# Cyan4973/FiniteStateEntropy

Hardware: NVIDIA H100
Metric: encode+decode GB/s (uncompressed) per GPU on 32 KB blocks; bit-exact vs ref (higher is better)
Workload: dtype u8

## Files before the change

finitestateentropy_b200/csrc/fse_dev.cuh:

```cuda
#pragma once
#include "common.cuh"

namespace fseb {

__device__ __forceinline__ unsigned hibit0(unsigned v) { return v ? hibit(v) : 0u; }

__device__ inline unsigned d_min_tablelog(u64 srcSize, unsigned msv)
{
    unsigned const bySrc = hibit0((u32)srcSize) + 1, bySym = hibit0(msv) + 2;
    return bySrc < bySym ? bySrc : bySym;
}

__device__ inline unsigned d_optimal_tablelog(unsigned maxTableLog, u64 srcSize, unsigned msv, unsigned minus)
{
    unsigned const bySrc = hibit0((u32)(srcSize - 1)) - minus;
    unsigned const floorBits = d_min_tablelog(srcSize, msv);
    unsigned tl = maxTableLog ? maxTableLog : FSE_DEF_TLOG;
    if (bySrc < tl) tl = bySrc;
    if (floorBits > tl) tl = floorBits;
    if (tl < FSE_MIN_TLOG) tl = FSE_MIN_TLOG;
    if (tl > FSE_MAX_TLOG) tl = FSE_MAX_TLOG;
    return tl;
}

// ... 149 lines not shown
            if (upto > *msvPtr) return err(E_MSV_TOO_SMALL);
            while (sym < upto) norm[sym++] = 0;
            if ((ip <= end - 7) || (ip + (held >> 3) <= end - 4)) { ip += held >> 3; held &= 7; bits = rd32(in + ip) >> held; }
            else bits >>= 2;
        }
        int const cut = (2 * threshold - 1) - remaining;
        int v;
        if ((bits & (u32)(threshold - 1)) < (u32)cut) { v = (int)(bits & (u32)(threshold - 1)); held += width - 1; }
        else { v = (int)(bits & (u32)(2 * threshold - 1)); if (v >= threshold) v -= cut; held += width; }
        v--;
        remaining -= v < 0 ? -v : v;
        norm[sym++] = (short)v;
        afterZero = !v;
        while (remaining < threshold) { width--; threshold >>= 1; }
        if ((ip <= end - 7) || (ip + (held >> 3) <= end - 4)) { ip += held >> 3; held &= 7; }
        else { held -= (int)(8 * (end - 4 - ip)); ip = end - 4; }
        bits = rd32(in + ip) >> (held & 31);
    }
    if (remaining != 1) return err(E_CORRUPT);
    if (held > 32) return err(E_CORRUPT);
    *msvPtr = sym - 1;
    ip += (held + 7) >> 3;
    if (padded && (u64)ip > trueSize) return err(E_CORRUPT);
    return (u64)ip;
}

__device__ inline bool d_spread_serial(u16* cellSym, const short* norm, unsigned msv, unsigned tl)
{
    u32 const size = 1u << tl, mask = size - 1;
    u32 const stride = (size >> 1) + (size >> 3) + 3;
    u32 high = size - 1, pos = 0;
    for (u32 s = 0; s <= msv; s++) if (norm[s] == -1) cellSym[high--] = (u16)s;
    for (u32 s = 0; s <= msv; s++) {
        int const n = norm[s];
        for (int k = 0; k < n; k++) {
            cellSym[pos] = (u16)s;
            do pos = (pos + stride) & mask; while (pos > high);
        }
    }
    return pos == 0;
}

__device__ inline void d_build_ctable_serial(u32* ct, const short* norm, unsigned msv, unsigned tl, u16* cellSym, u32* start)
{
    u32 const size = 1u << tl;
    u16* const hdr = (u16*)ct;
    u16* const next = hdr + 2;
    u32* const tt = ct + 1 + (tl ? (size >> 1) : 1);
    hdr[0] = (u16)tl; hdr[1] = (u16)msv;
    start[0] = 0;
    for (u32 s = 1; s <= msv + 1; s++) start[s] = start[s - 1] + (u32)(norm[s - 1] == -1 ? 1 : norm[s - 1]);
    start[msv + 1] = size + 1;
    d_spread_serial(cellSym, norm, msv, tl);
    for (u32 u = 0; u < size; u++) next[start[cellSym[u]]++] = (u16)(size + u);
    u32 total = 0;
    for (u32 s = 0; s <= msv; s++) {
        int const n = norm[s];
        if (n == 0) { tt[2 * s + 1] = ((tl + 1) << 16) - size; tt[2 * s] = 0; continue; }
        if (n == -1 || n == 1) { tt[2 * s + 1] = (tl << 16) - size; tt[2 * s] = total - 1; total++; }
        else {
            u32 const maxOut = tl - hibit((u32)n - 1);
            tt[2 * s + 1] = (maxOut << 16) - ((u32)n << maxOut);
            tt[2 * s] = total - (u32)n; total += (u32)n;
        }
    }
}

template <bool WIDE>
__device__ inline u64 d_build_dtable_serial(u32* dt, const short* norm, unsigned msv, unsigned tl,
                                            unsigned msvLimit, unsigned tlLimit, u16* cellSym, u16* nextOf)
{
    u32 const size = 1u << tl;
    unsigned fast = 1;
    if (msv > msvLimit) return err(E_MSV_TOO_LARGE);
    if (tl > tlLimit) return err(E_TLOG_TOO_LARGE);
    for (u32 s = 0; s <= msv; s++) {
        if (norm[s] == -1) nextOf[s] = 1;
        else { if (norm[s] >= (short)(1 << (tl - 1))) fast = 0; nextOf[s] = (u16)norm[s]; }
    }
    dt[0] = tl | (fast << 16);
    if (!d_spread_serial(cellSym, norm, msv, tl)) return err(E_GENERIC);
    for (u32 u = 0; u < size; u++) {
        u32 const sym = cellSym[u];
        u32 const x = nextOf[sym]++;
        u32 const nb = tl - hibit(x);
        u32 const ns = ((x << nb) - size) & 0xFFFF;
        dt[1 + u] = WIDE ? (ns | (nb << 16) | (sym << 20)) : (ns | (sym << 16) | (nb << 24));
    }
    return 0;
}

}
```

finitestateentropy_b200/csrc/huf_build_dev.cuh:

```cuda
#pragma once
#include "common.cuh"
#include "fse_dev.cuh"
#include "sink_dev.cuh"

namespace fseb {

struct HNode { u32 count; u16 parent; u8 sym; u8 len; };

struct HNodeView {
    HNode* p;
    __device__ u32 count(int i) const { return p[i].count; }
    __device__ u32 len(int i) const { return p[i].len; }
    __device__ void set_len(int i, u32 v) const { p[i].len = (u8)v; }
};
struct PackedNodeView {
    u32* p; int stride;
    __device__ u32 count(int i) const { return p[i * stride] & 0xFFFFFFu; }
    __device__ u32 len(int i) const { return p[i * stride] >> 24; }
    __device__ void set_len(int i, u32 v) const { u32& x = p[i * stride]; x = (x & 0xFFFFFFu) | (v << 24); }
};

template <class Nodes>
__device__ inline u32 d_huf_limit_depth(Nodes nd, u32 last, u32 maxBits)
{
    u32 const deepest = nd.len(last);
    if (deepest <= maxBits) return deepest;
    int debt = 0;
    u32 const unit = 1u << (deepest - maxBits);
    int n = (int)last;
    u32 const NONE = 0xF0F0F0F0u;
    u32 lastOfRank[HUF_MAX_TLOG + 2];
    while (nd.len(n) > maxBits) {
        debt += (int)(unit - (1u << (deepest - nd.len(n))));
        nd.set_len(n, maxBits); n--;
    }
    while (nd.len(n) == maxBits) n--;
    debt >>= (deepest - maxBits);
    for (u32 i = 0; i < HUF_MAX_TLOG + 2; i++) lastOfRank[i] = NONE;
    {   u32 cur = maxBits;
        for (int pos = n; pos >= 0; pos--) {
            if (nd.len(pos) >= cur) continue;
            cur = nd.len(pos);
            lastOfRank[maxBits - cur] = (u32)pos;
        }
    }
    while (debt > 0) {
        u32 dec = hibit((u32)debt) + 1;
        for (; dec > 1; dec--) {
            u32 const hi = lastOfRank[dec], lo = lastOfRank[dec - 1];
            if (hi == NONE) continue;
            if (lo == NONE) break;
            if (nd.count(hi) <= 2 * nd.count(lo)) break;
        }
        while (dec <= HUF_MAX_TLOG && lastOfRank[dec] == NONE) dec++;
        debt -= 1 << (dec - 1);
        if (lastOfRank[dec - 1] == NONE) lastOfRank[dec - 1] = lastOfRank[dec];
        nd.set_len(lastOfRank[dec], nd.len(lastOfRank[dec]) + 1);
        if (lastOfRank[dec] == 0) lastOfRank[dec] = NONE;
        else {
            lastOfRank[dec]--;
// ... 65 lines not shown
    u32 const mb = s_ret;
    if (mb > HUF_MAX_TLOG) return err(E_GENERIC);
    if ((u32)tid <= msv) lenOf[nd[tid].sym] = nd[tid].len;
    __syncthreads();
    if ((u32)tid <= msv) {
        u32 const len = lenOf[tid];
        u32 before = 0;
        for (u32 jj = 0; jj < (u32)tid; jj++) before += (lenOf[jj] == len);
        ctable[tid] = ((firstVal[len] + before) & 0xFFFF) | (len << 16);
    } else ctable[tid & 255] = 0;
    __syncthreads();
    return mb;
}

__device__ __forceinline__ void warp_sort256_desc(u32 (&key)[8], unsigned lane)
{
    #pragma unroll
    for (u32 k = 2; k <= 256; k <<= 1) {
        #pragma unroll
        for (u32 j = k >> 1; j > 0; j >>= 1) {
            if (j >= 32) {
                u32 const dj = j >> 5;
                #pragma unroll
                for (u32 i = 0; i < 8; i++) {
                    if (i & dj) continue;
                    u32 const e = i * 32;
                    bool const desc = (k == 256) || ((e & k) != 0) ;
                    u32 const lo = min(key[i], key[i | dj]), hi = max(key[i], key[i | dj]);
                    key[i] = desc ? hi : lo; key[i | dj] = desc ? lo : hi;
                }
            } else {
                #pragma unroll
                for (u32 i = 0; i < 8; i++) {
                    u32 const e = i * 32 + lane;
                    u32 const other = __shfl_xor_sync(0xFFFFFFFFu, key[i], j);
                    bool const asc = (k == 256) ? false : ((e & k) == 0);
                    bool const takeMin = ((e & j) == 0) == asc;
                    key[i] = takeMin ? min(key[i], other) : max(key[i], other);
                }
            }
        }
    }
}

__device__ inline u64 d_huf_compress_weights(u8* out, u64 cap, const u8* w, u64 n, u32* wksp)
{
    unsigned* const count = wksp;
    short* const norm = (short*)(wksp + 16);
    u32* const ct = wksp + 24;
    u16* const cellSym = (u16*)(wksp + 84);
    u32* const start = wksp + 116;
    unsigned msv = HUF_MAX_TLOG, tl = 6, best = 0;
    if (n <= 1) return 0;
    for (unsigned i = 0; i <= HUF_MAX_TLOG; i++) count[i] = 0;
    for (u64 i = 0; i < n; i++) count[w[i]]++;
    while (!count[msv]) msv--;
    for (unsigned s = 0; s <= msv; s++) best = count[s] > best ? count[s] : best;
    if (best == n) return 1;
    if (best == 1) return 0;
    tl = d_optimal_tablelog(tl, n, msv, 2);
    u64 r = d_normalize(norm, tl, count, n, msv); if (is_err(r)) return r;
    r = d_write_ncount(out, cap, norm, msv, tl); if (is_err(r)) return r;
    u64 const o = r;
    d_build_ctable_serial(ct, norm, msv, tl, cellSym, start);
    r = d_fse_encode_serial(out + o, cap - o, w, n, ct);
    if (r == 0) return 0;
    return o + r;
}

template <class CTable>
__device__ inline u64 d_huf_write_ctable(u8* out, u64 cap, CTable ctable, unsigned msv, unsigned huffLog, u32* wksp)
{
    u8* const weight = (u8*)(wksp + 160);
    if (msv > HUF_MAX_SV) return err(E_MSV_TOO_LARGE);
    for (unsigned n = 0; n < msv; n++) {
        unsigned const len = (ctable[n] >> 16) & 0xFF;
        weight[n] = (u8)(len ? huffLog + 1 - len : 0);
    }
    {   u64 const h = d_huf_compress_weights(out + 1, cap - 1, weight, msv, wksp);
        if (is_err(h)) return h;
        if ((h > 1) & (h < msv / 2)) { out[0] = (u8)h; return h + 1; }
    }
    if (msv > 128) return err(E_GENERIC);
    if (((msv + 1) / 2) + 1 > cap) return err(E_DST_TOO_SMALL);
    out[0] = (u8)(128 + (msv - 1));
    weight[msv] = 0;
    for (unsigned n = 0; n < msv; n += 2) out[(n / 2) + 1] = (u8)((weight[n] << 4) + weight[n + 1]);
    return ((msv + 1) / 2) + 1;
}

}
```

finitestateentropy_b200/csrc/huf_encode.cu:

```cuda
#include <mutex>
#include <type_traits>
#include <vector>
#include "common.cuh"
#include "launchers.h"
#include "launch_util.cuh"
#include "fse_dev.cuh"
#include "sink_dev.cuh"
#include "huf_build_dev.cuh"
#include "pack_dev.cuh"

namespace fseb {
namespace hufe {

constexpr unsigned FULL = 0xFFFFFFFFu;

struct __align__(16) Plan {
    u32 ctable[256];
    u8  header[136];
    u32 hSize;
    u32 state;
    u32 total;
    u32 streamOff[4];
    u32 streamBytes[4];
    u16 segCount[4][256];
};
enum : u32 { PLAN_EMIT = 0, PLAN_FINAL = 1, PLAN_EMIT_1X = 2 };

constexpr int PLAN_WARPS = 8;
constexpr u32 GROUP = 32;
constexpr u32 HDR_STRIDE = 34 + 224 + 1;
constexpr u32 CT_ROW = HDR_STRIDE;
constexpr u32 ROWS = CT_ROW + 256;
constexpr u32 NODE_END = 0x7FFFFFFFu, LEAF_END = 0xFFFFFFFFu;
struct PlanCta {
    u32 nd[ROWS][GROUP];
    u8  sym[256][GROUP];
    u64 res[GROUP];
    u16 msv[GROUP];
    u8  last[GROUP];
    u8  tlog[GROUP];
    u8  live[GROUP];
};
static_assert(ROWS >= 1 + 256 + PLAN_WARPS * 4 * 256 / GROUP, "segment histograms must fit in the rows above the leaves");
static_assert(ROWS >= 1 + 511 && CT_ROW >= 1 + 256, "node rows");
static_assert(HUF_BLOCK_MAX < (1u << 24), "node counts share a word with an 8-bit parent / length");
static_assert(sizeof(PlanCta) <= 76 * 1024, "three CTAs per SM");

template <int NS, class Count>
__device__ __forceinline__ void stream_bits(const u32 (&cell)[8], Count count, u32 (&bits)[NS])
{
    #pragma unroll
    for (int k = 0; k < NS; k++) {
        u32 acc = 0;
        #pragma unroll
        for (u32 i = 0; i < 8; i++) acc += count(k, i) * (cell[i] >> 16);
        #pragma unroll
        for (int dlt = 16; dlt; dlt >>= 1) acc += __shfl_xor_sync(FULL, acc, dlt);
        bits[k] = acc;
    }
}

template <int NS>
__device__ __forceinline__ bool place_streams(const u32 (&bits)[NS], u64 hs, u64 capLeft, u32 (&offs)[NS], u32 (&lens)[NS], u64& total)
{
    u64 op = (NS == 4) ? 6 : 0; bool fits = true;
    #pragma unroll
    for (int t = 0; t < NS; t++) {
        u64 const capk = capLeft - op;
        u64 const tot = (u64)bits[t] + 1;
        if (fits && (capk <= 8 || (tot >> 3) >= capk - 8)) fits = false;
        offs[t] = (u32)(hs + op); lens[t] = (u32)((tot + 7) >> 3);
        op += lens[t];
    }
    total = hs + op;
    return fits;
}

template <int NS, class Count>
__device__ __forceinline__ bool plan_streams(Plan& P, const u32 (&cell)[8], Count count, const u8* hdr, u64 hs, u64 cap, u32 n,
                                             unsigned lane, u64& total)
{
    u32 bits[NS], offs[NS], lens[NS];
    stream_bits<NS>(cell, count, bits);
// ... 54 lines not shown
    }
    for (u32 k = i + lane; k < end; k += 32) atomicAdd(&cnt[s[k]], 1u);
}

__device__ __forceinline__ void warp_hist4_pipelined(u32 (*count4)[256], const u8* s, u32 n, u32 seg, unsigned lane)
{
    const uint4* const gv = reinterpret_cast<const uint4*>(s) + lane;
    u32 const B = n / 2048, perSeg = seg / 2048;
    auto load = [&](uint4 (&x)[4], u32 b) {
        #pragma unroll
        for (int h = 0; h < 4; h++) x[h] = __ldg(gv + b * 128 + 32 * h);
    };
    auto count = [&](const uint4 (&x)[4], u32 b) {
        u32* const cnt = count4[b / perSeg];
        #pragma unroll
        for (int h = 0; h < 4; h++) {
            u32 const wd[4] = { x[h].x, x[h].y, x[h].z, x[h].w };
            #pragma unroll
            for (int k = 0; k < 4; k++) {
                u32 const y = wd[k];
                atomicAdd(&cnt[y & 0xFF], 1u); atomicAdd(&cnt[__byte_perm(y, 0, 0x4441)], 1u);
                atomicAdd(&cnt[__byte_perm(y, 0, 0x4442)], 1u); atomicAdd(&cnt[y >> 24], 1u);
            }
        }
    };
    uint4 xa[4], xb[4];
    load(xa, 0);
    #pragma unroll 1
    for (u32 b = 0; b < B; b += 2) {
        if (b + 1 < B) load(xb, b + 1);
        count(xa, b);
        if (b + 2 < B) load(xa, b + 2);
        if (b + 1 < B) count(xb, b + 1);
    }
}

template <class Geo, int NS>
__global__ void __launch_bounds__(32 * PLAN_WARPS, 3)
huf_plan_kernel(Geo g, u8* __restrict__ cbuf, u64* __restrict__ csizes, const u8* __restrict__ src,
                unsigned msvReq, unsigned tlogReq, Plan* __restrict__ plans)
{
    extern __shared__ __align__(16) unsigned char smem_raw[];
    PlanCta& S = *reinterpret_cast<PlanCta*>(smem_raw);
    unsigned const lane = threadIdx.x & 31u, warp = threadIdx.x >> 5;
    u32 const b0 = blockIdx.x * GROUP;
    constexpr bool REP = std::is_same_v<Geo, RepeatDescs>;
    constexpr bool CHAIN = std::is_base_of_v<ChainDescs, Geo>;
    static_assert(NS == 4 || NS == 1 || (NS == 0 && CHAIN), "4X, 1X, or mixed chains");
#define FSEB_FINAL(v) { if (lane == 0) {                                                                            \
        if constexpr (CHAIN) { g.fact[b].kind = CF_ARGS; g.fact[b].exitValue = (v); }                                  \
        else { P.state = 1; enc_out(g, csizes, b) = (v); }                                                             \
        S.live[c] = 0; } continue; }

    u32 (*const count4)[256] = reinterpret_cast<u32 (*)[256]>(&S.nd[257][0] + warp * 4 * 256);
    #pragma unroll 1
    for (u32 c = warp; c < GROUP; c += PLAN_WARPS) {
        __syncwarp();
        u32 const b = b0 + c;
        if (b >= g.nBlocks) { if (lane == 0) S.live[c] = 0; continue; }
        u32 const n = enc_len(g, b);
        u64 const cap = enc_cap(g, b);
        const u8* const s = enc_src(g, src, b);
        Plan& P = plans[b];
        if (!n) FSEB_FINAL(0);
        if (!cap) FSEB_FINAL(0);
        if (n > HUF_BLOCK_MAX) FSEB_FINAL(err(E_SRC_WRONG));
        if (tlogReq > HUF_MAX_TLOG) FSEB_FINAL(err(E_TLOG_TOO_LARGE));
        if (msvReq > HUF_MAX_SV) FSEB_FINAL(err(E_MSV_TOO_LARGE));
        unsigned const msvDecl = msvReq ? msvReq : HUF_MAX_SV;
        int flag = 0; bool prefer = false;
        if constexpr (REP) { flag = g.repeat[b]; prefer = g.prefer[b] != 0; }
        bool const oldNow = REP && prefer && flag == 2;

        u32 const seg = (n + 3) / 4;
        for (u32 i = lane; i < 4 * 256; i += 32) (&count4[0][0])[i] = 0;
        __syncwarp();
        if ((reinterpret_cast<u64>(s) & 15) == 0 && seg % 2048 == 0 && n == 4 * seg) warp_hist4_pipelined(count4, s, n, seg, lane);
        else {
            #pragma unroll 1
            for (u32 k = 0; k < 4; k++) {
                u32 const beg = min(k * seg, n), end = (k < 3) ? min((k + 1) * seg, n) : n;
                warp_hist_range(count4[k], s, beg, end, lane);
            }
        }
        __syncwarp();
        u32 cnt[8], top = 0, best = 0;
        #pragma unroll
        for (u32 i = 0; i < 8; i++) {
            u32 const sy = i * 32 + lane;
            cnt[i] = count4[0][sy] + count4[1][sy] + count4[2][sy] + count4[3][sy];
            if (cnt[i]) top = sy;
            best = max(best, cnt[i]);
        }
        #pragma unroll
        for (int dlt = 16; dlt; dlt >>= 1) { top = max(top, __shfl_xor_sync(FULL, top, dlt)); best = max(best, __shfl_xor_sync(FULL, best, dlt)); }
        if (!CHAIN && !oldNow) {
            if (msvDecl < 255 && top > msvDecl) FSEB_FINAL(err(E_MSV_TOO_SMALL));
            if (best == n) {
                if constexpr (!std::is_same_v<Geo, PackedDescs>) { if (lane == 0) enc_dst(g, cbuf, b)[0] = s[0]; }
                FSEB_FINAL(1);
            }
            if (best <= (n >> 7) + 4) FSEB_FINAL(0);
        }
        bool histExit = false;
        if constexpr (CHAIN) {
            bool const mst = msvReq != 0 && msvReq < 255 && top > msvReq;
            histExit = mst || best == n || best <= (n >> 7) + 4;
            if (lane == 0) {
                ChainFact& F = g.fact[b];
                F.kind = histExit ? CF_HIST : CF_TREE; F.msv = (u16)top;
                F.exitValue = mst ? err(E_MSV_TOO_SMALL) : best == n ? 1 : 0;
            }
        }
        u32 const msv = top;
        #pragma unroll
        for (u32 k = 0; k < 4; k++)
            #pragma unroll
            for (u32 i = 0; i < 8; i++) P.segCount[k][i * 32 + lane] = (u16)count4[k][i * 32 + lane];
        if (CHAIN && histExit) { if (lane == 0) S.live[c] = 0; continue; }
        if constexpr (REP) {
            if (!oldNow && flag == 1) {
                const u32* const old = g.ctable[b];
                bool bad = false;
                #pragma unroll
                for (u32 i = 0; i < 8; i++) { u32 const sy = i * 32 + lane; bad |= sy <= msv && cnt[i] && ((old[sy] >> 16) & 0xFFu) == 0; }
                if (__any_sync(FULL, bad)) { flag = 0; if (lane == 0) g.repeat[b] = 0; }
            }
            if (oldNow || (prefer && flag != 0)) {
                if (lane == 0) { S.msv[c] = (u16)msv; S.live[c] = 3; }
                continue;
            }
        }
        u32 key[8], nnz = 0;
        #pragma unroll
        for (u32 i = 0; i < 8; i++) { u32 const sy = i * 32 + lane; key[i] = ((sy <= msv ? cnt[i] : 0u) << 8) | (255u - sy); nnz += __popc(__ballot_sync(FULL, cnt[i] != 0)); }
        warp_sort256_desc(key, lane);
        #pragma unroll
        for (u32 i = 0; i < 8; i++) {
            u32 const r = i * 32 + lane;
            if (r <= msv) { S.nd[1 + r][c] = key[i] >> 8; S.sym[r][c] = (u8)(255u - (key[i] & 0xFFu)); }
        }
        if (lane == 0) {
            S.nd[0][c] = 0;
            S.msv[c] = (u16)msv; S.last[c] = (u8)(nnz - 1); S.live[c] = (REP && flag != 0) ? 2 : 1;
            S.tlog[c] = (u8)d_optimal_tablelog(tlogReq ? tlogReq : HUF_DEF_TLOG, n, msv, 1);
        }
    }
    __syncthreads();

    if (warp == 0) {
        u32 const c = lane;
        bool const live = REP ? (S.live[c] == 1 || S.live[c] == 2) : S.live[c];
        u32 const msv = S.msv[c];
        u32* const col = &S.nd[1][c];
        auto at = [&](int i) -> u32& { return col[i * (int)GROUP]; };
        u32* const ct = &S.nd[CT_ROW][c];
        u64 res = 0;
        if (live) {
            int const last = S.last[c];
            int fresh = 256, leaf = last, inner = fresh;
            int const root = fresh + leaf - 1;
            {   u32 const x = at(leaf), y = at(leaf - 1);
                at(fresh) = x + y;
                fresh++; leaf -= 2;
            }
            u32 cl = leaf >= 0 ? at(leaf) : LEAF_END, ci = at(inner);
            while (fresh <= root) {
                int a, bb; u32 ca, cb;
                if (cl < ci) { a = leaf--; ca = cl; cl = leaf >= 0 ? at(leaf) : LEAF_END; } else { a = inner++; ca = ci; ci = inner < fresh ? at(inner) : NODE_END; }
                if (cl < ci) { bb = leaf--; cb = cl; cl = leaf >= 0 ? at(leaf) : LEAF_END; } else { bb = inner++; cb = ci; ci = inner < fresh ? at(inner) : NODE_END; }
                u32 const sum = ca + cb;
                at(fresh) = sum;
                if (inner == fresh) ci = sum;
                u32 const tag = (u32)(fresh - 256) << 24;
                at(a) = ca | tag; at(bb) = cb | tag;
                fresh++;
            }
            at(root) &= 0xFFFFFFu;
            for (int m = root - 1; m >= 256; m--) { u32 const v = at(m); at(m) = (v & 0xFFFFFFu) | (((at(256 + (int)(v >> 24)) >> 24) + 1) << 24); }
            for (int m = 0; m <= last; m++) { u32 const v = at(m); at(m) = (v & 0xFFFFFFu) | (((at(256 + (int)(v >> 24)) >> 24) + 1) << 24); }
            u32 const mb = d_huf_limit_depth(PackedNodeView{ col, (int)GROUP }, (u32)last, S.tlog[c]);
            if (mb > HUF_MAX_TLOG) res = err(E_GENERIC);
            else {
                u32 perLen[HUF_MAX_TLOG + 1], nextVal[HUF_MAX_TLOG + 1];
                for (u32 i = 0; i <= HUF_MAX_TLOG; i++) { perLen[i] = 0; nextVal[i] = 0; }
                for (int m = 0; m <= last; m++) perLen[at(m) >> 24]++;
                u32 v = 0;
                for (int m = (int)mb; m > 0; m--) { nextVal[m] = v; v = (v + perLen[m]) >> 1; }
                for (u32 r = 0; r <= msv; r++) ct[S.sym[r][c] * GROUP] = (int)r <= last ? at((int)r) >> 24 : 0u;
                for (u32 sy = 0; sy <= msv; sy++) { u32 const len = ct[sy * GROUP]; ct[sy * GROUP] = (nextVal[len]++ & 0xFFFF) | (len << 16); }
                S.tlog[c] = (u8)mb;
            }
        }
        __syncwarp();
        if (live && !is_err(res)) {
            u64 const cap = enc_cap(g, b0 + c);
            u32* const area = &S.nd[0][0] + c * HDR_STRIDE;
            struct Col { const u32* p; __device__ u32 operator[](u32 i) const { return p[i * GROUP]; } };
            res = d_huf_write_ctable(reinterpret_cast<u8*>(area), cap < 136 ? cap : 136, Col{ ct }, msv, S.tlog[c], area + 34);
        }
        S.res[c] = res;
    }
    __syncthreads();

    #pragma unroll 1
    for (u32 c = warp; c < GROUP; c += PLAN_WARPS) {
        if (!S.live[c]) continue;
        u32 const b = b0 + c;
        u32 const n = enc_len(g, b);
        u64 const cap = enc_cap(g, b);
        Plan& P = plans[b];
        u64 hs = S.res[c];
        auto const count = [&](auto form, int k, u32 i) {
            u32 const sy = i * 32 + lane;
            return (decltype(form)::value == 4) ? (u32)P.segCount[k][sy] : (u32)P.segCount[0][sy] + P.segCount[1][sy] + P.segCount[2][sy] + P.segCount[3][sy];
        };
        auto const new_cells = [&](u32 (&cell)[8]) {
            u32 const msv = S.msv[c];
            #pragma unroll
            for (u32 i = 0; i < 8; i++) cell[i] = (i * 32 + lane <= msv) ? S.nd[CT_ROW + i * 32 + lane][c] : 0u;
        };
        auto const block_counts = [&](u32 (&sum)[8]) {
            #pragma unroll
            for (u32 i = 0; i < 8; i++) { u32 const sy = i * 32 + lane; sum[i] = (u32)P.segCount[0][sy] + P.segCount[1][sy] + P.segCount[2][sy] + P.segCount[3][sy]; }
        };
        const u8* const hdr = reinterpret_cast<const u8*>(&S.nd[0][0] + c * HDR_STRIDE);
        u32 cell[8];
        u64 total;
        auto const plan = [&](auto form) {
            return plan_streams<decltype(form)::value>(P, cell, [&](int k, u32 i) { return count(form, k, i); }, hdr, hs, cap, n, lane, total);
        };
        if constexpr (CHAIN) {
            ChainFact& F = g.fact[b];
            if (lane == 0) F.hSize = hs;
            if (is_err(hs) || hs + 12 >= n) continue;
            u32 sum[8];
            new_cells(cell);
            block_counts(sum);
            bool const ok = by_form<NS>(enc_single(g, b), plan);
            if (!ok) {
                #pragma unroll
                for (u32 i = 0; i < 8; i++) P.ctable[i * 32 + lane] = cell[i];
                if constexpr (std::is_same_v<Geo, ChainPackedLiteralsDescs>)
                    for (u32 i = lane; i < (u32)hs; i += 32) P.header[i] = hdr[i];
            }
            u32 const newBits = estimate_bits(cell, sum);
            if (lane == 0) { F.newBits = newBits; F.newValue = ok ? total : 0; }
            continue;
        }
        bool useOld = false;
        if constexpr (REP) useOld = S.live[c] == 3;
        if (!useOld) {
            if (is_err(hs)) FSEB_FINAL(hs);
            if constexpr (REP) {
                new_cells(cell);
                if (S.live[c] == 2) {
                    u32 old[8], sum[8];
                    #pragma unroll
                    for (u32 i = 0; i < 8; i++) old[i] = g.ctable[b][i * 32 + lane] & 0xFFFFFFu;
                    block_counts(sum);
                    useOld = (estimate_bits(old, sum) >> 3) <= hs + (estimate_bits(cell, sum) >> 3) || hs + 12 >= n;
                }
                if (!useOld && hs + 12 < n) {
                    #pragma unroll
                    for (u32 i = 0; i < 8; i++) g.ctable[b][i * 32 + lane] = cell[i];
                    if (lane == 0) g.repeat[b] = 0;
                }
            }
            if (!useOld && hs + 12 >= n) FSEB_FINAL(0);
        }
        if constexpr (REP) {
            if (useOld) {
                hs = 0;
                #pragma unroll
                for (u32 i = 0; i < 8; i++) cell[i] = g.ctable[b][i * 32 + lane] & 0xFFFFFFu;
            }
        } else new_cells(cell);
        if (!by_form<NS>(enc_single(g, b), plan)) FSEB_FINAL(0);
        if (lane == 0) { P.state = 0; enc_out(g, csizes, b) = total; }
    }
#undef FSEB_FINAL
}

constexpr int CHAIN_WARPS = 4;

__global__ void __launch_bounds__(1024)
huf_chain_check_kernel(const u64* __restrict__ start, u32 nChains, u32 nBlocks, u32* __restrict__ malformed)
{
    bool bad = threadIdx.x == 0 && (start[0] != 0 || start[nChains] != nBlocks);
    for (u64 c = threadIdx.x; c < nChains; c += blockDim.x) bad |= start[c + 1] < start[c];
    bad = __syncthreads_or(bad);
    if (threadIdx.x == 0) *malformed = bad;
}

struct ChainBlock {
    ChainFact f;
    u32 cnt[4][8];
    u32 cell[8];
    u8* dst;
    u64 cap;
    u32 n;
    int prefer;
};
struct ChainBlockMixed : ChainBlock {
    bool single;
};
template <class Geo, class Blk>
__device__ __forceinline__ void chain_load(const Geo& g, const Plan* plans, u32 b, Blk& x, unsigned lane)
{
    x.f = g.fact[b];
    const Plan& P = plans[b];
    #pragma unroll
    for (int k = 0; k < 4; k++)
        #pragma unroll
        for (u32 i = 0; i < 8; i++) x.cnt[k][i] = P.segCount[k][i * 32 + lane];
    #pragma unroll
    for (u32 i = 0; i < 8; i++) x.cell[i] = P.ctable[i * 32 + lane];
    if constexpr (std::is_same_v<Geo, ChainDescs> || std::is_same_v<Geo, ChainMixedDescs>) x.dst = enc_dst(g, nullptr, b);
    else x.dst = nullptr;
    x.cap = enc_cap(g, b); x.n = enc_len(g, b); x.prefer = g.prefer[b];
    if constexpr (std::is_same_v<Blk, ChainBlockMixed>) x.single = enc_single(g, b);
}

template <int S>
__device__ __forceinline__ bool chain_plan(Plan& P, const u32 (&T)[8], u64 hs, const ChainBlock& x, const u32 (&sum)[8], unsigned lane,
                                           u64& r)
{
    u32 const n = x.n;
    auto const count = [&](int k, u32 i) { return S == 4 ? x.cnt[k][i] : sum[i]; };
    u32 bits[S], offs[S], lens[S];
    u64 total;
    stream_bits<S>(T, count, bits);
    bool const fits = place_streams<S>(bits, hs, x.cap - hs, offs, lens, total);
    bool const ok = !(S == 4 && (x.cap - hs < 6 + 1 + 1 + 1 + 8 || n < 12)) && fits && total < (u64)n - 1;
// ... 625 lines not shown

cudaError_t launch_huf_encode(const BatchGeom& g, void* cbuf, u64* csizes, const void* src,
                              unsigned msv, unsigned tlog, cudaStream_t stream)
{
    return huf_encode<BatchGeom, 4>(g, cbuf, csizes, src, msv, tlog, stream);
}

template <class Geo>
static cudaError_t huf_encode_descs(const Geo& g, int nStreams, unsigned msv, unsigned tlog, cudaStream_t stream)
{
    return nStreams == 1 ? huf_encode<Geo, 1>(g, nullptr, nullptr, nullptr, msv, tlog, stream)
                         : huf_encode<Geo, 4>(g, nullptr, nullptr, nullptr, msv, tlog, stream);
}
cudaError_t launch_huf_encode_blocks(const BlockDescs& g, int nStreams, unsigned msv, unsigned tlog, cudaStream_t stream)
{
    return huf_encode_descs(g, nStreams, msv, tlog, stream);
}
cudaError_t launch_huf_encode_packed(const PackedDescs& g, int nStreams, unsigned msv, unsigned tlog, cudaStream_t stream)
{
    return huf_encode_descs(g, nStreams, msv, tlog, stream);
}
cudaError_t launch_huf_encode_repeat(const RepeatDescs& g, int nStreams, unsigned msv, unsigned tlog, cudaStream_t stream)
{
    return huf_encode_descs(g, nStreams, msv, tlog, stream);
}
cudaError_t launch_huf_encode_chains(const ChainDescs& g, int nStreams, unsigned msv, unsigned tlog, cudaStream_t stream)
{
    return huf_encode_descs(g, nStreams, msv, tlog, stream);
}
cudaError_t launch_huf_encode_chains_packed(const ChainPackedDescs& g, int nStreams, unsigned msv, unsigned tlog, cudaStream_t stream)
{
    return huf_encode_descs(g, nStreams, msv, tlog, stream);
}
cudaError_t launch_huf_encode_chains_mixed(const ChainMixedDescs& g, unsigned msv, unsigned tlog, cudaStream_t stream)
{
    return huf_encode<ChainMixedDescs, 0>(g, nullptr, nullptr, nullptr, msv, tlog, stream);
}
cudaError_t launch_huf_encode_chains_packed_mixed(const ChainPackedMixedDescs& g, unsigned msv, unsigned tlog, cudaStream_t stream)
{
    return huf_encode<ChainPackedMixedDescs, 0>(g, nullptr, nullptr, nullptr, msv, tlog, stream);
}
cudaError_t launch_huf_encode_literals_chains_packed(const ChainPackedLiteralsDescs& g, unsigned msv, unsigned tlog, cudaStream_t stream)
{
    return huf_encode<ChainPackedLiteralsDescs, 0>(g, nullptr, nullptr, nullptr, msv, tlog, stream);
}

cudaError_t launch_huf_chain_check(const u64* start, u32 nChains, u32 nBlocks, u32* malformed, cudaStream_t stream)
{
    hufe::huf_chain_check_kernel<<<1, 1024, 0, stream>>>(start, nChains, nBlocks, malformed);
    return cudaGetLastError();
}

}
```

finitestateentropy_b200/csrc/micro.cu:

```cuda
#include "common.cuh"
#include "launchers.h"
#include "fse_dev.cuh"
#include "bitsrc_dev.cuh"
#include "sink_dev.cuh"
#include "huf_dev.cuh"
#include "huf_build_dev.cuh"
#include "huf_x2_dev.cuh"
#include "micro.h"

namespace fseb {

__global__ void __launch_bounds__(256) hist_kernel(const u8* src, u64 n, u32 declared, u32* out , u64* ret)
{
    __shared__ u32 h[8][256];
    __shared__ u32 tot[256];
    int const tid = threadIdx.x;
    for (int i = tid; i < 8 * 256; i += 256) (&h[0][0])[i] = 0;
    __syncthreads();
    u32* const mine = h[tid >> 5];
    for (u64 i = tid; i < n; i += 256) atomicAdd(&mine[src[i]], 1u);
    __syncthreads();
    {   u32 c = 0; for (int w = 0; w < 8; w++) c += h[w][tid]; tot[tid] = c; }
    __syncthreads();
    if (tid == 0) {
// ... 22 lines not shown
    if (s_bad) { for (u32 i = tid; i <= declared; i += 256) out[i] = 0; if (tid == 0) *ret = err(E_MSV_TOO_SMALL); return; }
    u32 top = 0, best = 0;
    for (u32 i = tid; i <= declared; i += 256) { u32 const c = out[i]; if (c) { top = i; best = c > best ? c : best; } }
    atomicMax(&s_top, top); atomicMax(&s_best, best);
    __syncthreads();
    if (tid == 0) { out[declared + 1] = n ? s_top : 0; *ret = n ? s_best : 0; }
}

__global__ void __launch_bounds__(256) micro_kernel(int op, MicroArgs A, u8* buf, u64* ret)
{
    __shared__ u32 s_count[256];
    __shared__ u32 s_ct[256];
    __shared__ HNode s_nodes[2 * 256 + 2];
    __shared__ u32 s_a[256], s_b[256];
    __shared__ u32 s_w[384];
    int const tid = threadIdx.x;
    switch (op) {
    case MOP_NORMALIZE: {
        if (tid == 0) *ret = d_normalize((short*)(buf + MICRO_OUT), (unsigned)A.a[0], (const unsigned*)buf, A.a[1], (unsigned)A.a[2]);
        break; }
    case MOP_WRITE_NCOUNT: {
        if (tid == 0) *ret = d_write_ncount(buf + MICRO_OUT, A.a[0], (const short*)buf, (unsigned)A.a[1], (unsigned)A.a[2]);
        break; }
    case MOP_READ_NCOUNT: {
        if (tid == 0) {
            unsigned msv = (unsigned)A.a[1], tl = 0;
            *ret = d_read_ncount((short*)(buf + MICRO_OUT), &msv, &tl, buf, A.a[0]);
            ((u32*)(buf + MICRO_META))[0] = msv; ((u32*)(buf + MICRO_META))[1] = tl;
        }
        break; }
    case MOP_BUILD_CTABLE: {
        if (tid == 0) {
            unsigned const msv = (unsigned)A.a[0], tl = (unsigned)A.a[1];
            if (tl > 13 || msv > 4095) { *ret = err(E_TLOG_TOO_LARGE); break; }
            d_build_ctable_serial((u32*)(buf + MICRO_OUT), (const short*)buf, msv, tl, (u16*)(buf + MICRO_WORK), (u32*)(buf + MICRO_WORK + 32768));
            *ret = 0;
        }
        break; }
    case MOP_BUILD_DTABLE: {
        if (tid == 0) {
            unsigned const msv = (unsigned)A.a[0], tl = (unsigned)A.a[1];
            if (A.a[2]) *ret = d_build_dtable_serial<true>((u32*)(buf + MICRO_OUT), (const short*)buf, msv, tl, U16_MAX_SV, U16_MAX_TLOG, (u16*)(buf + MICRO_WORK), (u16*)(buf + MICRO_WORK + 32768));
            else *ret = d_build_dtable_serial<false>((u32*)(buf + MICRO_OUT), (const short*)buf, msv, tl, FSE_MAX_SV, FSE_MAX_TLOG, (u16*)(buf + MICRO_WORK), (u16*)(buf + MICRO_WORK + 32768));
        }
        break; }
    case MOP_HUF_BUILD_CTABLE: {
        s_count[tid] = ((u32)tid <= A.a[0]) ? ((const u32*)buf)[tid] : 0;
        __syncthreads();
        u64 const r = cta_huf_build_ctable(s_ct, s_count, (u32)A.a[0], (u32)A.a[1], s_nodes, s_a, s_b);
        if (!is_err(r)) ((u32*)(buf + MICRO_OUT))[tid] = s_ct[tid];
        if (tid == 0) *ret = r;
        break; }
    case MOP_HUF_WRITE_CTABLE: {
        if (tid == 0) *ret = d_huf_write_ctable(buf + MICRO_OUT, A.a[0] < 136 ? A.a[0] : 136, (const u32*)buf, (unsigned)A.a[1], (unsigned)A.a[2], s_w);
        break; }
    case MOP_HUF_READ_STATS: {
        if (tid == 0) {
            u32 nb = 0, tl = 0;
            *ret = d_huf_read_stats(buf + MICRO_OUT, A.a[1], (u32*)(buf + MICRO_META), &nb, &tl, buf, A.a[0]);
            ((u32*)(buf + MICRO_META_HUF))[0] = nb; ((u32*)(buf + MICRO_META_HUF))[1] = tl;
        }
        break; }
    case MOP_HUF_READ_DTABLE_X1: {
        if (tid == 0) {
            u8* const weights = buf + MICRO_OUT;
            u32 rank[17]; u32 nb = 0, tl = 0;
            u32* const dt = (u32*)(buf + MICRO_DTABLE_X1);
            u16* const cells = (u16*)(dt + 1);
            u64 const h = d_huf_read_stats(weights, 256, rank, &nb, &tl, buf, A.a[0]);
            u32 const hdr = (u32)A.a[1];
            dt[0] = hdr;
            if (is_err(h)) { *ret = h; break; }
            if (tl > (hdr & 0xFF) + 1) { *ret = err(E_TLOG_TOO_LARGE); break; }
            dt[0] = (hdr & 0xFF0000FFu) | (tl << 16);
            u32 next = 0;
            for (u32 n = 1; n < tl + 1; n++) { u32 const cur = next; next += rank[n] << (n - 1); rank[n] = cur; }
            for (u32 n = 0; n < nb; n++) {
                u32 const w = weights[n], span = (1u << w) >> 1, cell = n | ((tl + 1 - w) << 8);
                for (u32 u = 0; u < span; u++) cells[rank[w] + u] = (u16)cell;
                rank[w] += span;
            }
            *ret = h;
        }
        break; }
    case MOP_FSE_ENCODE_CT: {
        if (tid == 0) *ret = d_fse_encode_serial(buf + A.a[3], A.a[1], buf + A.a[2], A.a[0], (const u32*)buf);
        break; }
    case MOP_FSE_DECODE_DT: {
        if (tid == 0) *ret = d_fse_decode_serial(buf + A.a[3], A.a[1], buf + A.a[2], A.a[0], (const u32*)buf);
        break; }
    case MOP_HUF_ENCODE4X_CT: {
        __shared__ u64 s_len[4];
        const u32* const ct = (const u32*)buf;
        const u8* const in = buf + A.a[2]; u8* const out = buf + A.a[3];
        u64 const n = A.a[0], cap = A.a[1];
        u64 const seg = (n + 3) / 4;
        bool const refuse = cap < 6 + 1 + 1 + 1 + 8 || n < 12;
        u8* const stage = buf + A.a[3] + ((cap + 15) & ~15ull);
        if (tid < 4 && !refuse) {
            u64 const beg = seg * tid, end = tid < 3 ? seg * (tid + 1) : n;
            BitSink sk; sink_open(sk, stage + tid * ((cap + 15) & ~15ull), cap);
            for (u64 i = end; i-- > beg;) { u32 const e = ct[in[i]]; sink_put(sk, e & 0xFFFF, e >> 16); }
            sink_put(sk, 1, 1);
            s_len[tid] = sk.nbits;
            if (sk.held) { if (sk.nbytes < cap) sk.out[sk.nbytes] = (u8)sk.acc; }
        }
        __syncthreads();
        if (tid == 0) {
            if (refuse) { *ret = 0; break; }
            u64 op = 6; u64 r = 0; bool ok = true;
            for (int k = 0; k < 4 && ok; k++) {
                u64 const room = cap - op;
                u64 const bits = s_len[k], bytes = (bits + 7) >> 3;
                if (room <= 8 || (bits >> 3) >= room - 8) { ok = false; break; }
                const u8* const sp = stage + k * ((cap + 15) & ~15ull);
                for (u64 i = 0; i < bytes; i++) out[op + i] = sp[i];
                if (k < 3) { out[2 * k] = (u8)bytes; out[2 * k + 1] = (u8)(bytes >> 8); }
                op += bytes;
            }
            r = ok ? op : 0;
            *ret = r;
        }
        break; }
    case MOP_HUF_ENCODE1X_CT: {
        if (tid == 0) {
            const u32* const ct = (const u32*)buf; const u8* const in = buf + A.a[2];
            u64 const n = A.a[0], cap = A.a[1];
            if (cap < 8) { *ret = 0; break; }
            BitSink sk; sink_open(sk, buf + A.a[3], cap);
            if (!sk.usable) { *ret = 0; break; }
            for (u64 i = n; i-- > 0;) { u32 const e = ct[in[i]]; sink_put(sk, e & 0xFFFF, e >> 16); }
            *ret = sink_close(sk);
        }
        break; }
    case MOP_HUF_READ_DTABLE_X2: {
        if (tid == 0) *ret = d_huf_build_dtable_x2((u32*)(buf + MICRO_DTABLE_X2), (u32)A.a[1], buf + MICRO_OUT, buf + MICRO_META, buf + MICRO_META + 256, buf, A.a[0]);
        break; }
    case MOP_HUF_DECODE4X1_DT:
    case MOP_HUF_DECODE1X1_DT:
    case MOP_HUF_DECODE4X2_DT:
    case MOP_HUF_DECODE1X2_DT: {
        __shared__ u64 s_init[4]; __shared__ u32 s_done[4];
        bool const four = op == MOP_HUF_DECODE4X1_DT || op == MOP_HUF_DECODE4X2_DT;
        const u32* const dtab = (const u32*)buf; const u8* const c = buf + A.a[2]; u8* const out = buf + A.a[3];
        u64 const r = (op == MOP_HUF_DECODE4X1_DT || op == MOP_HUF_DECODE1X1_DT)
                    ? cta_huf_decode<d_huf_decode_stream_x1>(four, dtab, c, A.a[0], out, A.a[1], s_init, s_done)
                    : cta_huf_decode<d_huf_decode_stream_x2>(four, dtab, c, A.a[0], out, A.a[1], s_init, s_done);
        if (tid == 0) *ret = r;
        break; }
    default: if (tid == 0) *ret = err(E_GENERIC);
    }
}

cudaError_t launch_hist(const void* src, u64 n, u32 declared, u32* out, u64* ret, cudaStream_t s)
{ hist_kernel<<<1, 256, 0, s>>>((const u8*)src, n, declared, out, ret); return cudaGetLastError(); }
cudaError_t launch_hist16(const void* src, u64 n, u32 declared, u32* out, u64* ret, cudaStream_t s)
{ hist16_kernel<<<1, 256, 0, s>>>((const u16*)src, n, declared, out, ret); return cudaGetLastError(); }
cudaError_t launch_micro(int op, const MicroArgs& A, void* buf, u64* ret, cudaStream_t s)
// ... 4 lines not shown
```

finitestateentropy_b200/csrc/sink_dev.cuh:

```cuda
#pragma once
#include "common.cuh"

namespace fseb {

struct BitSink { u8* out; u64 cap; u64 acc; unsigned held; u64 nbytes; u64 nbits; bool usable; };

__device__ __forceinline__ void sink_open(BitSink& s, u8* dst, u64 cap)
{
    s.out = dst; s.cap = cap; s.acc = 0; s.held = 0; s.nbytes = 0; s.nbits = 0; s.usable = cap > 8;
}
__device__ __forceinline__ void sink_put(BitSink& s, u32 value, unsigned nb)
{
    if (nb == 0) return;
    s.acc |= ((u64)value & ((1ULL << nb) - 1)) << s.held;
    s.held += nb; s.nbits += nb;
    while (s.held >= 8) {
        if (s.nbytes < s.cap) s.out[s.nbytes] = (u8)s.acc;
        s.nbytes++; s.acc >>= 8; s.held -= 8;
    }
}
__device__ __forceinline__ u64 sink_close(BitSink& s)
{
    if (!s.usable) return 0;
    sink_put(s, 1, 1);
    if ((s.nbits >> 3) >= s.cap - 8) return 0;
    if (s.held) { s.out[s.nbytes] = (u8)s.acc; s.nbytes++; }
    return s.nbytes;
}

struct CtView { const u16* next; const u32* tt; unsigned tl; };
__device__ __forceinline__ CtView ct_view(const u32* ct)
{
    CtView v;
    v.tl = ((const u16*)ct)[0];
    v.next = ((const u16*)ct) + 2;
    v.tt = ct + 1 + (v.tl ? (1u << (v.tl - 1)) : 1);
    return v;
}
__device__ __forceinline__ u32 enc_seed(const CtView& c, u32 sym)
{
    u32 const dnb = c.tt[2 * sym + 1];
    u32 const nb = (dnb + (1u << 15)) >> 16;
    u32 const v = (nb << 16) - dnb;
    return c.next[(v >> nb) + c.tt[2 * sym]];
}
__device__ __forceinline__ u32 enc_step(BitSink& s, const CtView& c, u32 state, u32 sym)
{
    u32 const nb = (state + c.tt[2 * sym + 1]) >> 16;
    sink_put(s, state, nb);
    return c.next[(state >> nb) + c.tt[2 * sym]];
}

__device__ inline u64 d_fse_encode_serial(u8* dst, u64 cap, const u8* in, u64 n, const u32* ct)
{
    CtView const c = ct_view(ct);
    BitSink s;
    u32 st[2] = { 0, 0 }; bool seeded[2] = { false, false };
    if (n <= 2) return 0;
    sink_open(s, dst, cap);
    if (!s.usable) return 0;
    for (u64 i = n; i-- > 0;) {
        unsigned const k = (unsigned)(i & 1);
        if (!seeded[k]) { st[k] = enc_seed(c, in[i]); seeded[k] = true; }
        else st[k] = enc_step(s, c, st[k], in[i]);
    }
    sink_put(s, st[1], c.tl);
    sink_put(s, st[0], c.tl);
    return sink_close(s);
}

}
```

Before: 415.4.

## Streamline Huffman plan: length histogram, warp-parallel code assignment, faster bit sink

Several changes land together. The Huffman plan now packs per-length counts into a LenHist register pair, and code values are assigned warp-parallel with __match_any_sync instead of a serial per-lane loop. The weight-statistics histogram is derived from LenHist rather than recounted, and the depth-assignment and length-scatter loops are unrolled by 4. The bit sink now flushes 32 bits at a time instead of byte-by-byte, the FSE serial encoder is software-pipelined with the next symbol's table entries prefetched, and the ctable build prefetches the next cellSym. Optional clock64 instrumentation and a fixed-table debug mode are added behind macros that are off by default. Together these aim to cut serial per-thread latency in table building and header encoding, at the cost of more shared-memory layout coupling and a removed nb==0 guard in sink_put.

```diff
diff --git a/finitestateentropy_b200/csrc/fse_dev.cuh b/finitestateentropy_b200/csrc/fse_dev.cuh
--- a/finitestateentropy_b200/csrc/fse_dev.cuh
+++ b/finitestateentropy_b200/csrc/fse_dev.cuh
@@ -225,7 +225,12 @@
     for (u32 s = 1; s <= msv + 1; s++) start[s] = start[s - 1] + (u32)(norm[s - 1] == -1 ? 1 : norm[s - 1]);
     start[msv + 1] = size + 1;
     d_spread_serial(cellSym, norm, msv, tl);
-    for (u32 u = 0; u < size; u++) next[start[cellSym[u]]++] = (u16)(size + u);
+    u32 sym = cellSym[0];
+    for (u32 u = 0; u < size; u++) {
+        u32 const following = cellSym[(u + 1) & (size - 1)];
+        next[start[sym]++] = (u16)(size + u);
+        sym = following;
+    }
     u32 total = 0;
     for (u32 s = 0; s <= msv; s++) {
         int const n = norm[s];
diff --git a/finitestateentropy_b200/csrc/huf_build_dev.cuh b/finitestateentropy_b200/csrc/huf_build_dev.cuh
--- a/finitestateentropy_b200/csrc/huf_build_dev.cuh
+++ b/finitestateentropy_b200/csrc/huf_build_dev.cuh
@@ -3,9 +3,43 @@
 #include "fse_dev.cuh"
 #include "sink_dev.cuh"
 
+#ifndef FSEB200_HUFE_CLOCKS
+#define FSEB200_HUFE_CLOCKS 0
+#endif
+
 namespace fseb {
 
+#if FSEB200_HUFE_CLOCKS
+constexpr int PLAN_CLK_CTAS = 8192, PLAN_CLK_N = 16;
+static __device__ unsigned long long g_plan_clk[PLAN_CLK_CTAS][PLAN_CLK_N];
+__device__ __forceinline__ void plan_clock(int k)
+{
+    if (threadIdx.x != 0 || blockIdx.x >= (unsigned)PLAN_CLK_CTAS) return;
+    if (k == 0) for (int j = 1; j < PLAN_CLK_N; j++) g_plan_clk[blockIdx.x][j] = 0;
+    g_plan_clk[blockIdx.x][k] = clock64();
+}
+#define FSEB_PLAN_CLOCK(k) plan_clock(k)
+#else
+#define FSEB_PLAN_CLOCK(k) ((void)0)
+#endif
+
 struct HNode { u32 count; u16 parent; u8 sym; u8 len; };
+
+struct LenHist {
+    u64 lo = 0, hi = 0;
+    __device__ __forceinline__ void add(u32 len)
+    {
+        bool const low = len <= 7;
+        u64 const one = 1ull << (9 * (low ? len - 1 : len - 8));
+        lo += low ? one : 0; hi += low ? 0 : one;
+    }
+    __device__ __forceinline__ u32 get(u32 len) const
+    {
+        bool const low = len <= 7;
+        return (u32)(((low ? lo : hi) >> (9 * (low ? len - 1 : len - 8))) & 511u);
+    }
+};
+static_assert(HUF_MAX_TLOG == 12, "LenHist holds lengths 1 .. 12");
 
 struct HNodeView {
     HNode* p;
@@ -177,8 +211,6 @@
     u32* const start = wksp + 116;
     unsigned msv = HUF_MAX_TLOG, tl = 6, best = 0;
     if (n <= 1) return 0;
-    for (unsigned i = 0; i <= HUF_MAX_TLOG; i++) count[i] = 0;
-    for (u64 i = 0; i < n; i++) count[w[i]]++;
     while (!count[msv]) msv--;
     for (unsigned s = 0; s <= msv; s++) best = count[s] > best ? count[s] : best;
     if (best == n) return 1;
@@ -187,14 +219,17 @@
     u64 r = d_normalize(norm, tl, count, n, msv); if (is_err(r)) return r;
     r = d_write_ncount(out, cap, norm, msv, tl); if (is_err(r)) return r;
     u64 const o = r;
+    FSEB_PLAN_CLOCK(6);
     d_build_ctable_serial(ct, norm, msv, tl, cellSym, start);
+    FSEB_PLAN_CLOCK(7);
     r = d_fse_encode_serial(out + o, cap - o, w, n, ct);
+    FSEB_PLAN_CLOCK(8);
     if (r == 0) return 0;
     return o + r;
 }
 
 template <class CTable>
-__device__ inline u64 d_huf_write_ctable(u8* out, u64 cap, CTable ctable, unsigned msv, unsigned huffLog, u32* wksp)
+__device__ inline u64 d_huf_write_ctable(u8* out, u64 cap, CTable ctable, unsigned msv, unsigned huffLog, LenHist perLen, u32* wksp)
 {
     u8* const weight = (u8*)(wksp + 160);
     if (msv > HUF_MAX_SV) return err(E_MSV_TOO_LARGE);
@@ -202,6 +237,17 @@
         unsigned const len = (ctable[n] >> 16) & 0xFF;
         weight[n] = (u8)(len ? huffLog + 1 - len : 0);
     }
+    {   u32* const count = wksp;
+        u32 coded = 0;
+        for (unsigned i = 0; i <= HUF_MAX_TLOG; i++) count[i] = 0;
+        #pragma unroll
+        for (u32 len = 1; len <= HUF_MAX_TLOG; len++)
+            if (len <= huffLog) { u32 const k = perLen.get(len); count[huffLog + 1 - len] = k; coded += k; }
+        unsigned const lastLen = (ctable[msv] >> 16) & 0xFF;
+        if (lastLen - 1 < huffLog) { count[huffLog + 1 - lastLen]--; coded--; }
+        count[0] = msv - coded;
+    }
+    FSEB_PLAN_CLOCK(12);
     {   u64 const h = d_huf_compress_weights(out + 1, cap - 1, weight, msv, wksp);
         if (is_err(h)) return h;
         if ((h > 1) & (h < msv / 2)) { out[0] = (u8)h; return h + 1; }
diff --git a/finitestateentropy_b200/csrc/huf_encode.cu b/finitestateentropy_b200/csrc/huf_encode.cu
--- a/finitestateentropy_b200/csrc/huf_encode.cu
+++ b/finitestateentropy_b200/csrc/huf_encode.cu
@@ -26,9 +26,14 @@
 };
 enum : u32 { PLAN_EMIT = 0, PLAN_FINAL = 1, PLAN_EMIT_1X = 2 };
 
+#ifndef FSEB200_HUFE_TREE
+#define FSEB200_HUFE_TREE 1
+#endif
+
 constexpr int PLAN_WARPS = 8;
 constexpr u32 GROUP = 32;
 constexpr u32 HDR_STRIDE = 34 + 224 + 1;
+constexpr u32 LENHIST_AT = 34 + 140;
 constexpr u32 CT_ROW = HDR_STRIDE;
 constexpr u32 ROWS = CT_ROW + 256;
 constexpr u32 NODE_END = 0x7FFFFFFFu, LEAF_END = 0xFFFFFFFFu;
@@ -189,6 +194,7 @@
         else { P.state = 1; enc_out(g, csizes, b) = (v); }                                                             \
         S.live[c] = 0; } continue; }
 
+    FSEB_PLAN_CLOCK(0);
     u32 (*const count4)[256] = reinterpret_cast<u32 (*)[256]>(&S.nd[257][0] + warp * 4 * 256);
     #pragma unroll 1
     for (u32 c = warp; c < GROUP; c += PLAN_WARPS) {
@@ -284,6 +290,7 @@
         }
     }
     __syncthreads();
+    FSEB_PLAN_CLOCK(1);
 
     if (warp == 0) {
         u32 const c = lane;
@@ -293,7 +300,16 @@
         auto at = [&](int i) -> u32& { return col[i * (int)GROUP]; };
         u32* const ct = &S.nd[CT_ROW][c];
         u64 res = 0;
+        LenHist perLen;
+#if !FSEB200_HUFE_TREE
         if (live) {
+            for (u32 sy = 0; sy <= msv; sy++) { ct[sy * GROUP] = 8u << 16; perLen.add(8); }
+            S.tlog[c] = 8;
+        }
+        if (false) {
+#else
+        if (live) {
+#endif
             int const last = S.last[c];
             int fresh = 256, leaf = last, inner = fresh;
             int const root = fresh + leaf - 1;
@@ -313,32 +329,53 @@
                 at(a) = ca | tag; at(bb) = cb | tag;
                 fresh++;
             }
+            FSEB_PLAN_CLOCK(2);
             at(root) &= 0xFFFFFFu;
             for (int m = root - 1; m >= 256; m--) { u32 const v = at(m); at(m) = (v & 0xFFFFFFu) | (((at(256 + (int)(v >> 24)) >> 24) + 1) << 24); }
-            for (int m = 0; m <= last; m++) { u32 const v = at(m); at(m) = (v & 0xFFFFFFu) | (((at(256 + (int)(v >> 24)) >> 24) + 1) << 24); }
+            for (int m = 0; m <= last; m += 4) {
+                u32 v[4], up[4];
+                #pragma unroll
+                for (int j = 0; j < 4; j++) v[j] = at(m + j);
+                #pragma unroll
+                for (int j = 0; j < 4; j++) up[j] = at(256 + (int)(v[j] >> 24));
+                #pragma unroll
+                for (int j = 0; j < 4; j++) if (m + j <= last) at(m + j) = (v[j] & 0xFFFFFFu) | (((up[j] >> 24) + 1) << 24);
+            }
+            FSEB_PLAN_CLOCK(3);
             u32 const mb = d_huf_limit_depth(PackedNodeView{ col, (int)GROUP }, (u32)last, S.tlog[c]);
+            FSEB_PLAN_CLOCK(4);
             if (mb > HUF_MAX_TLOG) res = err(E_GENERIC);
             else {
-                u32 perLen[HUF_MAX_TLOG + 1], nextVal[HUF_MAX_TLOG + 1];
-                for (u32 i = 0; i <= HUF_MAX_TLOG; i++) { perLen[i] = 0; nextVal[i] = 0; }
-                for (int m = 0; m <= last; m++) perLen[at(m) >> 24]++;
-                u32 v = 0;
-                for (int m = (int)mb; m > 0; m--) { nextVal[m] = v; v = (v + perLen[m]) >> 1; }
-                for (u32 r = 0; r <= msv; r++) ct[S.sym[r][c] * GROUP] = (int)r <= last ? at((int)r) >> 24 : 0u;
-                for (u32 sy = 0; sy <= msv; sy++) { u32 const len = ct[sy * GROUP]; ct[sy * GROUP] = (nextVal[len]++ & 0xFFFF) | (len << 16); }
+                for (int r = 0; r <= last; r += 4) {
+                    u32 len[4], sy[4];
+                    #pragma unroll
+                    for (int j = 0; j < 4; j++) { int const q = min(r + j, last); len[j] = at(q) >> 24; sy[j] = S.sym[q][c]; }
+                    #pragma unroll
+                    for (int j = 0; j < 4; j++) if (r + j <= last) { ct[sy[j] * GROUP] = len[j] << 16; perLen.add(len[j]); }
+                }
+                for (u32 r = last + 1; r <= msv; r++) ct[S.sym[r][c] * GROUP] = 0;
                 S.tlog[c] = (u8)mb;
             }
+            FSEB_PLAN_CLOCK(5);
         }
         __syncwarp();
         if (live && !is_err(res)) {
             u64 const cap = enc_cap(g, b0 + c);
             u32* const area = &S.nd[0][0] + c * HDR_STRIDE;
+            u32* const lens = area + LENHIST_AT;
+            lens[0] = (u32)perLen.lo; lens[1] = (u32)(perLen.lo >> 32); lens[2] = (u32)perLen.hi; lens[3] = (u32)(perLen.hi >> 32);
             struct Col { const u32* p; __device__ u32 operator[](u32 i) const { return p[i * GROUP]; } };
-            res = d_huf_write_ctable(reinterpret_cast<u8*>(area), cap < 136 ? cap : 136, Col{ ct }, msv, S.tlog[c], area + 34);
+#if FSEB200_HUFE_TREE
+            res = d_huf_write_ctable(reinterpret_cast<u8*>(area), cap < 136 ? cap : 136, Col{ ct }, msv, S.tlog[c], perLen, area + 34);
+#else
+            res = 64; (void)cap;
+#endif
+            FSEB_PLAN_CLOCK(9);
         }
         S.res[c] = res;
     }
     __syncthreads();
+    FSEB_PLAN_CLOCK(10);
 
     #pragma unroll 1
     for (u32 c = warp; c < GROUP; c += PLAN_WARPS) {
@@ -353,9 +390,29 @@
             return (decltype(form)::value == 4) ? (u32)P.segCount[k][sy] : (u32)P.segCount[0][sy] + P.segCount[1][sy] + P.segCount[2][sy] + P.segCount[3][sy];
         };
         auto const new_cells = [&](u32 (&cell)[8]) {
-            u32 const msv = S.msv[c];
+            u32 const msv = S.msv[c], mb = S.tlog[c];
+            u32* const h = &S.nd[0][0] + c * HDR_STRIDE + LENHIST_AT;
+            LenHist perLen;
+            perLen.lo = h[0] | (u64)h[1] << 32; perLen.hi = h[2] | (u64)h[3] << 32;
+            u32 mine = 0, v = 0;
             #pragma unroll
-            for (u32 i = 0; i < 8; i++) cell[i] = (i * 32 + lane <= msv) ? S.nd[CT_ROW + i * 32 + lane][c] : 0u;
+            for (u32 k = HUF_MAX_TLOG; k >= 1; k--) { if (k == lane) mine = v; if (k <= mb) v = (v + perLen.get(k)) >> 1; }
+            __syncwarp();
+            if (lane <= HUF_MAX_TLOG) h[4 + lane] = mine;
+            __syncwarp();
+            u32 const before = (1u << lane) - 1;
+            #pragma unroll
+            for (u32 i = 0; i < 8; i++) {
+                u32 const sy = i * 32 + lane;
+                bool const in = sy <= msv;
+                u32 const len = in ? S.nd[CT_ROW + sy][c] >> 16 : 0xFFu;
+                u32 const same = __match_any_sync(FULL, len);
+                u32 const val = in ? h[4 + len] + __popc(same & before) : 0u;
+                __syncwarp();
+                if (in && (same >> lane) == 1u) h[4 + len] += __popc(same);
+                __syncwarp();
+                cell[i] = in ? (val & 0xFFFF) | (len << 16) : 0u;
+            }
         };
         auto const block_counts = [&](u32 (&sum)[8]) {
             #pragma unroll
@@ -417,6 +474,11 @@
         if (lane == 0) { P.state = 0; enc_out(g, csizes, b) = total; }
     }
 #undef FSEB_FINAL
+#if FSEB200_HUFE_CLOCKS
+    __syncthreads();
+    FSEB_PLAN_CLOCK(11);
+    if (threadIdx.x == 0 && blockIdx.x < (unsigned)PLAN_CLK_CTAS) { u32 sm; asm volatile("mov.u32 %0, %%smid;" : "=r"(sm)); g_plan_clk[blockIdx.x][15] = sm; }
+#endif
 }
 
 constexpr int CHAIN_WARPS = 4;
@@ -1148,3 +1210,15 @@
 }
 
 }
+
+#if FSEB200_HUFE_CLOCKS
+extern "C" __attribute__((visibility("default"))) size_t FSEB200_debug_plan_clocks(unsigned long long* host, size_t n)
+{
+    size_t const k = n < (size_t)fseb::PLAN_CLK_CTAS ? n : (size_t)fseb::PLAN_CLK_CTAS;
+    if (cudaMemcpyFromSymbol(host, fseb::g_plan_clk, k * fseb::PLAN_CLK_N * sizeof(unsigned long long)) != cudaSuccess) return 0;
+    return k;
+}
+#endif
+#if !FSEB200_HUFE_TREE
+extern "C" __attribute__((visibility("default"))) int FSEB200_debug_fixed_table(void) { return 1; }
+#endif
diff --git a/finitestateentropy_b200/csrc/micro.cu b/finitestateentropy_b200/csrc/micro.cu
--- a/finitestateentropy_b200/csrc/micro.cu
+++ b/finitestateentropy_b200/csrc/micro.cu
@@ -98,7 +98,12 @@
         if (tid == 0) *ret = r;
         break; }
     case MOP_HUF_WRITE_CTABLE: {
-        if (tid == 0) *ret = d_huf_write_ctable(buf + MICRO_OUT, A.a[0] < 136 ? A.a[0] : 136, (const u32*)buf, (unsigned)A.a[1], (unsigned)A.a[2], s_w);
+        if (tid == 0) {
+            const u32* const ct = (const u32*)buf;
+            LenHist perLen;
+            for (u32 n = 0; n <= (u32)A.a[1] && n <= HUF_MAX_SV; n++) { u32 const len = (ct[n] >> 16) & 0xFF; if (len - 1 < HUF_MAX_TLOG) perLen.add(len); }
+            *ret = d_huf_write_ctable(buf + MICRO_OUT, A.a[0] < 136 ? A.a[0] : 136, ct, (unsigned)A.a[1], (unsigned)A.a[2], perLen, s_w);
+        }
         break; }
     case MOP_HUF_READ_STATS: {
         if (tid == 0) {
@@ -148,8 +153,8 @@
             BitSink sk; sink_open(sk, stage + tid * ((cap + 15) & ~15ull), cap);
             for (u64 i = end; i-- > beg;) { u32 const e = ct[in[i]]; sink_put(sk, e & 0xFFFF, e >> 16); }
             sink_put(sk, 1, 1);
-            s_len[tid] = sk.nbits;
-            if (sk.held) { if (sk.nbytes < cap) sk.out[sk.nbytes] = (u8)sk.acc; }
+            s_len[tid] = sink_bits(sk);
+            sink_drain(sk);
         }
         __syncthreads();
         if (tid == 0) {
diff --git a/finitestateentropy_b200/csrc/sink_dev.cuh b/finitestateentropy_b200/csrc/sink_dev.cuh
--- a/finitestateentropy_b200/csrc/sink_dev.cuh
+++ b/finitestateentropy_b200/csrc/sink_dev.cuh
@@ -3,28 +3,35 @@
 
 namespace fseb {
 
-struct BitSink { u8* out; u64 cap; u64 acc; unsigned held; u64 nbytes; u64 nbits; bool usable; };
+struct BitSink { u8* out; u64 cap; u64 acc; unsigned held; u64 nbytes; bool usable; };
 
 __device__ __forceinline__ void sink_open(BitSink& s, u8* dst, u64 cap)
 {
-    s.out = dst; s.cap = cap; s.acc = 0; s.held = 0; s.nbytes = 0; s.nbits = 0; s.usable = cap > 8;
+    s.out = dst; s.cap = cap; s.acc = 0; s.held = 0; s.nbytes = 0; s.usable = cap > 8;
+}
+__device__ __forceinline__ void sink_store(BitSink& s, unsigned bytes)
+{
+    for (unsigned k = 0; k < bytes; k++) if (s.nbytes + k < s.cap) s.out[s.nbytes + k] = (u8)(s.acc >> (8 * k));
+    s.nbytes += bytes;
 }
 __device__ __forceinline__ void sink_put(BitSink& s, u32 value, unsigned nb)
 {
-    if (nb == 0) return;
     s.acc |= ((u64)value & ((1ULL << nb) - 1)) << s.held;
-    s.held += nb; s.nbits += nb;
-    while (s.held >= 8) {
-        if (s.nbytes < s.cap) s.out[s.nbytes] = (u8)s.acc;
-        s.nbytes++; s.acc >>= 8; s.held -= 8;
-    }
+    s.held += nb;
+    if (s.held >= 32) { sink_store(s, 4); s.acc >>= 32; s.held -= 32; }
+}
+__device__ __forceinline__ u64 sink_bits(const BitSink& s) { return 8 * s.nbytes + s.held; }
+__device__ __forceinline__ void sink_drain(BitSink& s)
+{
+    sink_store(s, (s.held + 7) / 8);
+    s.acc = 0; s.held = 0;
 }
 __device__ __forceinline__ u64 sink_close(BitSink& s)
 {
     if (!s.usable) return 0;
     sink_put(s, 1, 1);
-    if ((s.nbits >> 3) >= s.cap - 8) return 0;
-    if (s.held) { s.out[s.nbytes] = (u8)s.acc; s.nbytes++; }
+    if ((sink_bits(s) >> 3) >= s.cap - 8) return 0;
+    sink_drain(s);
     return s.nbytes;
 }
 
@@ -44,28 +51,25 @@
     u32 const v = (nb << 16) - dnb;
     return c.next[(v >> nb) + c.tt[2 * sym]];
 }
-__device__ __forceinline__ u32 enc_step(BitSink& s, const CtView& c, u32 state, u32 sym)
-{
-    u32 const nb = (state + c.tt[2 * sym + 1]) >> 16;
-    sink_put(s, state, nb);
-    return c.next[(state >> nb) + c.tt[2 * sym]];
-}
 
 __device__ inline u64 d_fse_encode_serial(u8* dst, u64 cap, const u8* in, u64 n, const u32* ct)
 {
     CtView const c = ct_view(ct);
     BitSink s;
-    u32 st[2] = { 0, 0 }; bool seeded[2] = { false, false };
     if (n <= 2) return 0;
     sink_open(s, dst, cap);
     if (!s.usable) return 0;
-    for (u64 i = n; i-- > 0;) {
-        unsigned const k = (unsigned)(i & 1);
-        if (!seeded[k]) { st[k] = enc_seed(c, in[i]); seeded[k] = true; }
-        else st[k] = enc_step(s, c, st[k], in[i]);
+    u32 cur = enc_seed(c, in[n - 1]), other = enc_seed(c, in[n - 2]);
+    u32 sym = in[n - 3];
+    u32 delta = c.tt[2 * sym], dnb = c.tt[2 * sym + 1];
+    for (u64 i = n - 2; i-- > 0;) {
+        u32 const x = cur, d = delta, nb = (x + dnb) >> 16;
+        if (i) { sym = in[i - 1]; delta = c.tt[2 * sym]; dnb = c.tt[2 * sym + 1]; }
+        sink_put(s, x, nb);
+        cur = other; other = c.next[(x >> nb) + d];
     }
-    sink_put(s, st[1], c.tl);
-    sink_put(s, st[0], c.tl);
+    sink_put(s, cur, c.tl);
+    sink_put(s, other, c.tl);
     return sink_close(s);
 }
 
```

Measured after the change: 420.1, median of 6. 1.1% higher.
